# 0xPabloxx/3d-pointcloud-orientation-estimation

Measured on AMD Instinct MI355X. Metric: clouds/sec fwd+bwd, pointnet_pp_vonMises N=1024, higher is better.
Workload: dtype f32; 1 GPU; configs[1]: models/pointnet_pp_vonMises.py single-peak KL, N=1024, batch=32 per GPU, fwd+loss+bwd+allreduce+Adam, random-init weights (seed 42), device-side centre sampling; per_gpu_batch=32, global_batch=32, points=1024, parallelism=single, launch=hipGraph(fwd+loss+bwd) + eager all-reduce/Adam (the update clears the gradients)

## Files before the change

### 3d-pointcloud-orientation-estimation_amd/csrc/gemm_kernels.hip

```cpp
#include <stdlib.h>

#include "kernels.h"

namespace pnpp {

static bool mid_tiles_on() {
    static int cached = -1;
    if (cached < 0) {
        const char *v = getenv("PNPP_NO_MID");
        cached = (v && atoi(v) != 0) ? 0 : 1;
    }
    return cached != 0;
}

constexpr int KC = 32;
constexpr int APITCH = KC + 1;

struct RawA {
    float4 p, q;
    int4 ia;
};

template <int MODE>
__device__ __forceinline__ RawA fetch_a4(const AOperand &A, int row, int k, int M, int Kd) {
// ... 1052 lines not shown
                        }
                        if constexpr (DEFER) held = acc[i][j], held_m0 = m0;
                        if constexpr (EMODE == E_STORE_STATS) s1[j] += (double)t1, s2[j] += (double)t2;
                        if constexpr (EMODE == E_STORE_STATS) {
                            if (E.pool_ext) {
                                const float sg = pool_sg[j];
                                float mx = sg * acc[i][j][0];
#pragma unroll
                                for (int r = 1; r < 16; ++r) mx = fmaxf(mx, sg * acc[i][j][r]);
                                mx = fmaxf(mx, __shfl_xor(mx, 32, 64));
                                int a = 64;
#pragma unroll
                                for (int r = 15; r >= 0; --r) a = (sg * acc[i][j][r] == mx) ? (r & 3) + 8 * (r >> 2) + 4 * lh : a;
                                a = min(a, __shfl_xor(a, 32, 64));
                                if constexpr (DEFER) {
                                    held_ext = sg * mx, held_arg = a;
                                } else if (lh == 0) {
                                    const size_t gi = (size_t)((m0 + wm * TM + i * 32) >> 5) * E.ldc + (n0 + wn * TN + j * 32 + l31);
                                    E.pool_ext[gi] = sg * mx;
                                    E.pool_arg[gi] = a;
                                }
                            }
                        }
                    }
            }
        }
        if constexpr (EMODE == E_MASK_STATS && NT == 1) {
            if (m0 + BM <= M && n0 + BN <= Nout) {
                done = true;
#pragma unroll
                for (int i = 0; i < MT; ++i)
#pragma unroll
                    for (int j = 0; j < NT; ++j) {
                        const int col = n0 + wn * TN + j * 32 + l31;
                        const float sc = E.scale[col], sh = E.shift[col], mu = E.mu[col], is = E.istd[col];
                        float *tb = E.c + (size_t)(m0 + wm * TM + i * 32) * E.ldc + (n0 + wn * TN + j * 32);
                        const unsigned lo = (unsigned)(4 * lh) * (unsigned)E.ldc + (unsigned)l31;
                        float *apb = Ap + (wm * TM + i * 32 + 4 * lh) * BN + wn * TN + j * 32 + l31;
                        float t1 = 0.f, t2 = 0.f;
#pragma unroll
                        for (int r = 0; r < 16; ++r) {
                            const float z0 = zp[i][j][r];
                            const float a0 = fmaf(z0, sc, sh);
                            const float v = a0 > 0.f ? acc[i][j][r] : 0.f;
                            float *tr = tb + (size_t)((r & 3) + 8 * (r >> 2)) * E.ldc;
                            if (!PNPP_WS_EXP_NO_STORE) tr[lo] = v;
                            t1 += v;
                            t2 = fmaf(v, (z0 - mu) * is, t2);
                            if constexpr (FDW) apb[((r & 3) + 8 * (r >> 2)) * BN] = fmaxf(a0, 0.f);
                        }
                        s1[j] += (double)t1, s2[j] += (double)t2;
                    }
            }
        }
        if (!done)
#pragma unroll
        for (int i = 0; i < MT; ++i)
#pragma unroll
            for (int j = 0; j < NT; ++j) {
                const int col = n0 + wn * TN + j * 32 + l31;
                float sc = 0.f, sh = 0.f, mu = 0.f, is = 0.f;
                if constexpr (EMODE == E_MASK_STATS) {
                    const int cc = min(col, Nout - 1);
                    sc = E.scale[cc], sh = E.shift[cc], mu = E.mu[cc], is = E.istd[cc];
                }
                float t1 = 0.f, t2 = 0.f;
#pragma unroll
                for (int r = 0; r < 16; ++r) {
                    const int row = m0 + wm * TM + i * 32 + (r & 3) + 8 * (r >> 2) + 4 * lh;
                    const bool ok = row < M && col < Nout;
                    float v = ok ? acc[i][j][r] : 0.f;
                    if constexpr (EMODE == E_STORE_STATS) {
                        t1 += v;
                        t2 = fmaf(v, v, t2);
                    } else if constexpr (EMODE == E_MASK_STATS) {
                        const float z0 = zp[i][j][r];
                        v = (fmaf(z0, sc, sh) > 0.f) ? v : 0.f;
                        t1 += v;
                        t2 = fmaf(v, (z0 - mu) * is, t2);
                    }
                    if (ok) E.c[(size_t)row * E.ldc + col] = v;
                    if constexpr (FDW) {
                        const int rl = wm * TM + i * 32 + (r & 3) + 8 * (r >> 2) + 4 * lh;
                        Ap[rl * BN + wn * TN + j * 32 + l31] = fmaxf(fmaf(zp[i][j][r], sc, sh), 0.f);
                    }
                }
                if constexpr (EMODE != E_STORE) s1[j] += (double)t1, s2[j] += (double)t2;
            }
        PNPP_STAMP(5)
        if constexpr (FDW) {
            __syncthreads();
            PNPP_STAMP(6)
            static_assert(4 % (BN / 32) == 0, "a wave's dW tiles must share their activation columns");
            constexpr int MC = BM / 32;
            const int kt = wave % (BN / 32);
            int colx[DT];
#pragma unroll
            for (int t = 0; t < DT; ++t) colx[t] = (((wave + 4 * t) / (BN / 32)) * 32 + l31) ^ (lh << 2);
            const float *abase = As + lh * KP, *bbase = Ap + lh * BN + kt * 32 + l31;
            float da[2][MC][DT], db[2][MC];
            auto ld = [&](int buf, int t2) {
                const int F = (t2 & 7) << 3;
                const float *pb = bbase + 2 * t2 * BN;
#pragma unroll
                for (int c = 0; c < MC; ++c) db[buf][c] = pb[32 * c * BN];
#pragma unroll
                for (int t = 0; t < DT; ++t) {
                    const float *pa = abase + 2 * t2 * KP + (colx[t] ^ F);
#pragma unroll
                    for (int c = 0; c < MC; ++c) da[buf][c][t] = pa[32 * c * KP];
                }
            };
            auto mm = [&](int buf) {
#pragma unroll
                for (int c = 0; c < MC; ++c)
#pragma unroll
                    for (int t = 0; t < DT; ++t)
                        dwacc[t] = PNPP_WS_MFMA(da[buf][c][t], db[buf][c], dwacc[t]);
            };
            if constexpr (KD >= PNPP_WS_DWTABLE_MINK || TUNED_128) {
                const float *pre[DT][8];
#pragma unroll
                for (int t = 0; t < DT; ++t)
#pragma unroll
                    for (int f = 0; f < 8; ++f) pre[t][f] = abase + 2 * f * KP + (colx[t] ^ (f << 3));
                auto ldt = [&](int buf, int t2) {
                    const int f = t2 & 7, h = t2 >> 3;
                    const float *pb = bbase + 2 * t2 * BN;
#pragma unroll
                    for (int c = 0; c < MC; ++c) db[buf][c] = pb[32 * c * BN];
#pragma unroll
                    for (int t = 0; t < DT; ++t) {
                        const float *pa = pre[t][f] + 16 * h * KP;
#pragma unroll
                        for (int c = 0; c < MC; ++c) da[buf][c][t] = pa[32 * c * KP];
                    }
                };
                ldt(0, 0);
#pragma unroll
                for (int t2 = 0; t2 < 16; t2 += 2) {
                    ldt(1, t2 + 1);
                    mm(0);
                    if (t2 + 2 < 16) ldt(0, t2 + 2);
                    mm(1);
                }
            } else {
                ld(0, 0);
#pragma unroll 1
                for (int t2 = 0; t2 < 16; t2 += 2) {
                    ld(1, t2 + 1);
                    mm(0);
                    if (t2 + 2 < 16) ld(0, t2 + 2);
                    mm(1);
                }
            }
            PNPP_STAMP(7)
        }
    }

    flush_held();
    PNPP_STAMP(9)
    if constexpr (FDW) {
      if (n0 + BN <= Nout) {
        float *wb = E.dwslab + (size_t)worker * KD * E.dw_ld + n0;
        const unsigned lo = (unsigned)(4 * lh) * (unsigned)E.dw_ld + (unsigned)l31;
#pragma unroll
        for (int t = 0; t < DT; ++t) {
            const int tile_id = wave + 4 * t, ct = tile_id / (BN / 32), kt = tile_id % (BN / 32);
            float *tb = wb + (size_t)(ct * 32) * E.dw_ld + kt * 32;
#pragma unroll
            for (int r = 0; r < 16; ++r) tb[(size_t)((r & 3) + 8 * (r >> 2)) * E.dw_ld + lo] = dwacc[t][r];
        }
      } else
#pragma unroll
        for (int t = 0; t < DT; ++t) {
            const int tile_id = wave + 4 * t, ct = tile_id / (BN / 32), kt = tile_id % (BN / 32);
#pragma unroll
            for (int r = 0; r < 16; ++r) {
                const int c = ct * 32 + (r & 3) + 8 * (r >> 2) + 4 * lh, k = n0 + kt * 32 + l31;
                if (k < Nout) E.dwslab[((size_t)worker * KD + c) * E.dw_ld + k] = dwacc[t][r];
            }
        }
    }

    if constexpr (EMODE != E_STORE) {
        __syncthreads();
        double *red = reinterpret_cast<double *>(lds);
#pragma unroll
        for (int j = 0; j < NT; ++j) {
            double a = s1[j] + shfl_xor_f64(s1[j], 32);
            double b = s2[j] + shfl_xor_f64(s2[j], 32);
            if (lh == 0) {
                const int cl = wn * TN + j * 32 + l31;
                red[(wm * 2 + 0) * BN + cl] = a;
                red[(wm * 2 + 1) * BN + cl] = b;
            }
        }
        __syncthreads();
        for (int f = tid; f < 2 * BN; f += 256) {
            const int which = f / BN, cl = f % BN;
            double t = 0.0;
#pragma unroll
            for (int w = 0; w < WM; ++w) t += red[(w * 2 + which) * BN + cl];
            if (n0 + cl < Nout) E.slab[((size_t)worker * 2 + which) * Nout + n0 + cl] = t;
        }
    }
    PNPP_STAMP(10)
}

template <int KD, int BM, int BN, int WM, int WN, int AM, int EM, bool FDW>
static int launch_ws_one(const AOperand &A, const BOperand &B, int M, int Nout, const Epilogue &E, int *nslab, hipStream_t st,
                         int *dw_slabs) {
    const int tiles = cdiv(M, BM), ncol = cdiv(Nout, BN);
    size_t lds = ((size_t)KD * BN + (size_t)BM * (KD % 32 == 0 ? KD : KD + 1) + (FDW ? (size_t)BM * BN : 0)) * sizeof(float);
    const size_t red_bytes = (size_t)WM * 2 * BN * sizeof(double);
    if (lds < red_bytes) lds = red_bytes;
    int per_cu = (int)((160 * 1024) / lds);
    if (per_cu > 3) per_cu = 3;
    if (per_cu < 1) per_cu = 1;
    int workers = (256 * per_cu) / ncol;
    if (workers > tiles) workers = tiles;
    if (workers > kMaxStatBlocks) workers = kMaxStatBlocks;
    if (workers < 1) workers = 1;
    if (nslab) *nslab = workers;
    if (dw_slabs) *dw_slabs = FDW ? workers : 0;
    ProfScope ps(st, "gemm_ws_kernel<%d,%d,%d,A%d,E%d%s> M=%d N=%d K=%d grid=%dx1", KD, BM, BN, AM, EM, FDW ? ",dW" : "", M, Nout,
                 KD, workers * ncol);
    auto kfn = gemm_ws_kernel<KD, BM, BN, WM, WN, AM, EM, FDW>;
    static size_t lds_granted = 0;
    if (lds > 48 * 1024 && lds > lds_granted) {
        (void)hipFuncSetAttribute((const void *)kfn, hipFuncAttributeMaxDynamicSharedMemorySize, (int)lds);
        lds_granted = lds;
    }
    hipLaunchKernelGGL(kfn, dim3(workers * ncol), dim3(256), lds, st, A, B, M, Nout, ncol, E);
    PNPP_CHECK_LAUNCH("gemm_ws");
    return PNPP_OK;
}

template <int KD, int BM, int BN, int WM, int WN, int AM>
static int launch_ws_e(const AOperand &A, const BOperand &B, int M, int Nout, const Epilogue &E, int *nslab, hipStream_t st,
                       int *dw_slabs = nullptr) {
    if (dw_slabs) *dw_slabs = 0;
    switch (E.mode) {
        case E_STORE: return launch_ws_one<KD, BM, BN, WM, WN, AM, E_STORE, false>(A, B, M, Nout, E, nslab, st, nullptr);
        case E_STORE_STATS: return launch_ws_one<KD, BM, BN, WM, WN, AM, E_STORE_STATS, false>(A, B, M, Nout, E, nslab, st, nullptr);
        case E_MASK_STATS:
            if constexpr ((AM == A_DZ || AM == A_DZ_POOL) && KD % 32 == 0 && ((KD / 32) * (BN / 32)) % 4 == 0) {
                if (E.dwslab && dw_slabs)
                    return launch_ws_one<KD, BM, BN, WM, WN, AM, E_MASK_STATS, true>(A, B, M, Nout, E, nslab, st, dw_slabs);
            }
            return launch_ws_one<KD, BM, BN, WM, WN, AM, E_MASK_STATS, false>(A, B, M, Nout, E, nslab, st, nullptr);
    }
    set_error("gemm_ws: bad epilogue mode %d", E.mode);
    return PNPP_ERR_ARG;
}

template <int KD, int BM, int BN, int WM, int WN>
static int launch_ws_dense(const AOperand &A, const BOperand &B, int M, int Nout, const Epilogue &E, int *nslab, hipStream_t st,
                           int *dw_slabs) {
    switch (A.mode) {
        case A_PLAIN: return launch_ws_e<KD, BM, BN, WM, WN, A_PLAIN>(A, B, M, Nout, E, nslab, st);
        case A_BNRELU: return launch_ws_e<KD, BM, BN, WM, WN, A_BNRELU>(A, B, M, Nout, E, nslab, st);
        case A_DZ: return launch_ws_e<KD, BM, BN, WM, WN, A_DZ>(A, B, M, Nout, E, nslab, st, dw_slabs);
        case A_DZ_POOL: return launch_ws_e<KD, BM, BN, WM, WN, A_DZ_POOL>(A, B, M, Nout, E, nslab, st, dw_slabs);
    }
    set_error("gemm_ws: bad A mode %d", A.mode);
    return PNPP_ERR_ARG;
}

static bool try_launch_ws(const AOperand &A, const BOperand &B, int M, int Nout, int Kd, const Epilogue &E, int *nslab,
                          hipStream_t st, int *rc, int *dw_slabs) {
    if (M < 8192 || Nout % 64 != 0) return false;
    const bool grouped = A.mode == A_GATHER || A.mode == A_CONCAT;
    if (grouped) {
        if (Kd != A.D + 4) return false;
        if (A.mode != A_GATHER) return false;
        if (A.D == 0) {
            if (Nout % 128 == 0) *rc = launch_ws_e<4, 128, 128, 4, 1, A_GATHER>(A, B, M, Nout, E, nslab, st);
            else *rc = launch_ws_e<4, 128, 64, 4, 1, A_GATHER>(A, B, M, Nout, E, nslab, st);
            return true;
        }
        if (A.D == 128 && ((uintptr_t)A.a & 15) == 0) {
            *rc = launch_ws_e<132, 64, 64, 2, 2, A_GATHER>(A, B, M, Nout, E, nslab, st);
            return true;
        }
        return false;
    }
    if (A.lda % 4 != 0 || ((uintptr_t)A.a & 15) != 0) return false;
    if (Kd == 64) {
        *rc = launch_ws_dense<64, 64, 64, 2, 2>(A, B, M, Nout, E, nslab, st, dw_slabs);
        return true;
    }
    if (Kd == 128) {
        *rc = launch_ws_dense<128, 64, 64, 2, 2>(A, B, M, Nout, E, nslab, st, dw_slabs);
        return true;
    }
    if (Kd == 256) {
        *rc = launch_ws_dense<256, 64, 64, 2, 2>(A, B, M, Nout, E, nslab, st, dw_slabs);
        return true;
    }
    return false;
}

template <int AMODE, int EMODE, bool BT, int NW>
__device__ __forceinline__ void gemm_smallm_body(const AOperand &A, const BOperand &B, int M, int Nout, int Kd, const Epilogue &E,
                                                 int bx, int by, int nblocks) {
    constexpr int NTHR = NW * 64, NJ = 1024 / NTHR;
    __shared__ __attribute__((aligned(16))) float lds[2 * NW * 32 * APITCH];
    const int tid = threadIdx.x, lane = tid & 63, wave = tid >> 6, l31 = lane & 31, lh = lane >> 5;
    float *As = lds + wave * 32 * APITCH;
    float *Ws = lds + (NW + wave) * 32 * APITCH;
    float *part = lds;
    const float *__restrict__ Bm = B.b;
    const int ldb = B.ldb;
    const int n0 = bx * 32, m0 = by * 32;
    const int nchunks = (Kd + KC - 1) / KC;
    const bool bvec = (ldb & 3) == 0 && ((uintptr_t)Bm & 15) == 0 && B.perm_D < 0 && B.rows >= 4 && (B.rows & 3) == 0;

    f32x16 acc;
#pragma unroll
    for (int r = 0; r < 16; ++r) acc[r] = 0.f;

    float p_g = 1.f, p_b = 0.f, p_bias = 0.f, p_rm = 0.f, p_rv = 0.f;
    unsigned long long p_sid = 0ull;
    if constexpr (EMODE == E_BN_APPLY) {
        const BnTail &T = E.bn;
        if (tid < 32 && n0 + tid < Nout) {
            const int c = n0 + tid;
            if (T.gamma) p_g = T.gamma[c];
            if (T.beta) p_b = T.beta[c];
            if (T.bias) p_bias = T.bias[c];
            if (T.rm) p_rm = T.rm[c], p_rv = T.rv[c];
        }
        if (T.mask_out) p_sid = T.rng_counter[0];
    }

    RawA na[4];
    float4 nw[4];
    float nb[KC / 2];
    auto fetch = [&](int c) {
        const int k0 = c * KC;
#pragma unroll
        for (int i = 0; i < 4; ++i) {
            const int r = (lane >> 3) + 8 * i, k = k0 + 4 * (lane & 7);
            na[i] = fetch_a4<AMODE>(A, m0 + r, k, M, Kd);
            if constexpr (BT) {
                const float *wrow = Bm + (size_t)min(n0 + r, Nout - 1) * ldb;
                if (bvec) {
                    nw[i] = *reinterpret_cast<const float4 *>(wrow + min(k, B.rows - 4));
                } else {
                    float t[4];
#pragma unroll
                    for (int e = 0; e < 4; ++e) {
                        const int kp = min(k + e, B.rows - 1);
                        t[e] = wrow[B.perm_D >= 0 ? (kp < B.perm_D ? kp + 3 : kp - B.perm_D) : kp];
                    }
                    nw[i] = make_float4(t[0], t[1], t[2], t[3]);
                }
            }
        }
        if constexpr (!BT) {
#pragma unroll
            for (int s2 = 0; s2 < KC / 2; ++s2) {
                const int k = k0 + 2 * s2 + lh;
                const float v = Bm[(size_t)min(k, B.rows - 1) * ldb + min(n0 + l31, Nout - 1)];
                nb[s2] = v * ((k < B.rows && n0 + l31 < Nout) ? 1.f : 0.f);
            }
        }
    };
    if (wave < nchunks) fetch(wave);
    for (int c = wave; c < nchunks; c += NW) {
        float cb[KC / 2];
        const int k0 = c * KC;
#pragma unroll
        for (int i = 0; i < 4; ++i) {
            const int r = (lane >> 3) + 8 * i, k = k0 + 4 * (lane & 7);
            const int o = r * APITCH + 4 * (lane & 7);
            float v[4];
            xform_a4<AMODE>(A, na[i], m0 + r, k, M, Kd, v);
            As[o] = v[0], As[o + 1] = v[1], As[o + 2] = v[2], As[o + 3] = v[3];
            if constexpr (BT) {
                const bool okw = n0 + r < Nout;
                Ws[o] = (okw && k < B.rows) ? nw[i].x : 0.f;
                Ws[o + 1] = (okw && k + 1 < B.rows) ? nw[i].y : 0.f;
                Ws[o + 2] = (okw && k + 2 < B.rows) ? nw[i].z : 0.f;
                Ws[o + 3] = (okw && k + 3 < B.rows) ? nw[i].w : 0.f;
            }
        }
        if constexpr (!BT) {
#pragma unroll
            for (int s2 = 0; s2 < KC / 2; ++s2) cb[s2] = nb[s2];
        }
        if (c + NW < nchunks) fetch(c + NW);
#pragma unroll
        for (int s2 = 0; s2 < KC / 2; ++s2) {
            const float bv = BT ? Ws[l31 * APITCH + 2 * s2 + lh] : cb[s2];
            acc = __builtin_amdgcn_mfma_f32_32x32x2f32(As[l31 * APITCH + 2 * s2 + lh], bv, acc, 0, 0, 0);
        }
    }
#pragma unroll
    for (int r = 0; r < 16; ++r) part[wave * 32 * APITCH + ((r & 3) + 8 * (r >> 2) + 4 * lh) * 32 + l31] = acc[r];
    __syncthreads();
    float v[NJ], w2[NJ];
#pragma unroll
    for (int j = 0; j < NJ; ++j) {
        const int e = tid + NTHR * j;
        v[j] = 0.f;
#pragma unroll
        for (int w = 0; w < NW; w += 4)
            v[j] += (part[w * 32 * APITCH + e] + part[(w + 1) * 32 * APITCH + e]) +
                    (part[(w + 2) * 32 * APITCH + e] + part[(w + 3) * 32 * APITCH + e]);
        w2[j] = 0.f;
    }
    __syncthreads();
#pragma unroll
    for (int j = 0; j < NJ; ++j) {
        const int e = tid + NTHR * j, row = m0 + e / 32, col = n0 + e % 32;
        const bool ok = row < M && col < Nout;
        float x = ok ? v[j] : 0.f;
        if constexpr (EMODE == E_MASK_STATS) {
            const int cc = min(col, Nout - 1);
            const float zp = E.zp[(size_t)min(row, M - 1) * E.ldc + cc];
            x = (fmaf(zp, E.scale[cc], E.shift[cc]) > 0.f) ? x : 0.f;
            w2[j] = x * ((zp - E.mu[cc]) * E.istd[cc]);
            part[1024 + e] = w2[j];
        }
        part[e] = x;
        if (ok) E.c[(size_t)row * E.ldc + col] = x;
    }
    if constexpr (EMODE == E_BN_APPLY) {
        const BnTail &T = E.bn;
        float *cs = part + 2048;
        __syncthreads();
        if (tid < 32 && n0 + tid < Nout) {
            const int c = n0 + tid;
            double s1 = 0.0, s2 = 0.0;
            for (int r = 0; r < 32; ++r) {
                const double x = (double)part[r * 32 + tid];
                s1 += x;
                s2 += x * x;
            }
            const double count = (double)M;
            const double mu = s1 / count;
            double var = s2 / count - mu * mu;
            if (var < 0.0) var = 0.0;
            const double is = 1.0 / sqrt(var + (double)T.eps);
            const double g = (double)p_g, bt = (double)p_b;
            const float sc = (float)(g * is), sh = (float)(bt - mu * g * is);
            T.mean[c] = (float)mu;
            T.istd[c] = (float)is;
            T.scale[c] = sc;
            T.shift[c] = sh;
            cs[tid] = sc;
            cs[32 + tid] = sh;
            if (T.rm) {
                const double bmean = mu + (double)p_bias;
                const double unbiased = count > 1.0 ? var * count / (count - 1.0) : var;
                T.rm[c] = (float)((1.0 - (double)T.momentum) * (double)p_rm + (double)T.momentum * bmean);
                T.rv[c] = (float)((1.0 - (double)T.momentum) * (double)p_rv + (double)T.momentum * unbiased);
            }
        }
        if (T.nbt && bx == 0 && tid == 0) *T.nbt += 1;
        __syncthreads();
#pragma unroll
        for (int j = 0; j < NJ; ++j) {
            const int e = tid + NTHR * j, row = m0 + e / 32, col = n0 + e % 32;
            if (row < M && col < Nout) {
                float y = fmaf(part[e], cs[e % 32], cs[32 + e % 32]);
                if (T.relu) y = fmaxf(y, 0.f);
                if (T.mask) y = T.mask[(size_t)row * E.ldc + col] ? y * T.drop_scale : 0.f;
                if (T.mask_out) {
                    const unsigned long long sid = p_sid;
                    const unsigned idx = (unsigned)(row * E.ldc + col);
                    unsigned c0 = idx, c1 = 0x44524f50u , c2 = (unsigned)sid, c3 = (unsigned)(sid >> 32);
                    unsigned k0 = (unsigned)T.rng_seed, k1 = (unsigned)(T.rng_seed >> 32);
#pragma unroll
                    for (int rd = 0; rd < 10; ++rd) {
                        const unsigned long long p0 = (unsigned long long)0xD2511F53u * c0, p1 = (unsigned long long)0xCD9E8D57u * c2;
                        const unsigned n0 = (unsigned)(p1 >> 32) ^ c1 ^ k0, n1 = (unsigned)p1, n2 = (unsigned)(p0 >> 32) ^ c3 ^ k1, n3 = (unsigned)p0;
                        c0 = n0, c1 = n1, c2 = n2, c3 = n3;
                        k0 += 0x9E3779B9u, k1 += 0xBB67AE85u;
                    }
                    const bool keep = (double)c0 >= (double)T.drop_p * 4294967296.0;
                    T.mask_out[(size_t)row * E.ldc + col] = keep ? 1 : 0;
                    y = keep ? y * T.drop_scale : 0.f;
                }
                T.y[(size_t)row * E.ldc + col] = y;
            }
        }
        if (T.mask_out) {
            __syncthreads();
            if (tid == 0) {
                const unsigned long long t = atomicAdd(&T.rng_counter[1], 1ull);
                if (t == (unsigned long long)nblocks - 1) {
                    T.rng_counter[1] = 0ull;
                    T.rng_counter[0] += 1ull;
                }
            }
        }
    } else if constexpr (EMODE != E_STORE) {
        __syncthreads();
        if (tid < 32 && n0 + tid < Nout) {
            double s1 = 0.0, s2 = 0.0;
            for (int r = 0; r < 32; ++r) {
                const double x = (double)part[r * 32 + tid];
                s1 += x;
                if constexpr (EMODE == E_STORE_STATS) s2 += x * x;
                else s2 += (double)part[1024 + r * 32 + tid];
            }
            E.slab[((size_t)by * 2 + 0) * Nout + n0 + tid] = s1;
            E.slab[((size_t)by * 2 + 1) * Nout + n0 + tid] = s2;
        }
    }
}

template <int AMODE, int EMODE, bool BT, int NW>
__global__ void __launch_bounds__(NW * 64)
gemm_smallm_kernel(const AOperand A, const BOperand B, int M, int Nout, int Kd, const Epilogue E) {
    gemm_smallm_body<AMODE, EMODE, BT, NW>(A, B, M, Nout, Kd, E, blockIdx.x, blockIdx.y, gridDim.x * gridDim.y);
}

template <int AM, int EM>
static void launch_smallm_t(const AOperand &A, const BOperand &B, int M, int Nout, int Kd, const Epilogue &E, dim3 grid,
                            hipStream_t st) {
    if constexpr (AM == A_PLAIN) {
        if (grid.y == 1 && Kd >= 256) {
            if (B.trans) hipLaunchKernelGGL((gemm_smallm_kernel<AM, EM, true, 16>), grid, dim3(1024), 0, st, A, B, M, Nout, Kd, E);
            else hipLaunchKernelGGL((gemm_smallm_kernel<AM, EM, false, 16>), grid, dim3(1024), 0, st, A, B, M, Nout, Kd, E);
            return;
        }
    }
    if (B.trans) hipLaunchKernelGGL((gemm_smallm_kernel<AM, EM, true, 4>), grid, dim3(256), 0, st, A, B, M, Nout, Kd, E);
    else hipLaunchKernelGGL((gemm_smallm_kernel<AM, EM, false, 4>), grid, dim3(256), 0, st, A, B, M, Nout, Kd, E);
}
template <int AM>
static int launch_smallm_e(const AOperand &A, const BOperand &B, int M, int Nout, int Kd, const Epilogue &E, dim3 grid,
                           hipStream_t st) {
    switch (E.mode) {
        case E_STORE: launch_smallm_t<AM, E_STORE>(A, B, M, Nout, Kd, E, grid, st); return PNPP_OK;
        case E_STORE_STATS: launch_smallm_t<AM, E_STORE_STATS>(A, B, M, Nout, Kd, E, grid, st); return PNPP_OK;
        case E_MASK_STATS: launch_smallm_t<AM, E_MASK_STATS>(A, B, M, Nout, Kd, E, grid, st); return PNPP_OK;
        case E_BN_APPLY:
            if constexpr (AM == A_PLAIN) {
                PNPP_REQUIRE(grid.y == 1 && E.bn.mean && E.bn.istd && E.bn.scale && E.bn.shift && E.bn.y, PNPP_ERR_ARG,
                             "gemm(small M): the BatchNorm epilogue needs all rows in one tile (M <= 32) and its outputs");
                launch_smallm_t<AM, E_BN_APPLY>(A, B, M, Nout, Kd, E, grid, st);
                return PNPP_OK;
            }
            break;
    }
    set_error("gemm(small M): bad epilogue mode %d", E.mode);
    return PNPP_ERR_ARG;
}

template <int BM, int BN, int WM, int WN>
static int launch_gemm_cfg(const AOperand &A, const BOperand &B, int M, int Nout, int Kd, const Epilogue &E, int *nslab,
                           hipStream_t st) {
    const int tiles = cdiv(M, BM);
    const int gx = tiles < kMaxStatBlocks ? tiles : kMaxStatBlocks;
    const dim3 grid(gx, cdiv(Nout, BN)), block(WM * WN * 64);
    if (nslab) *nslab = gx;
    ProfScope ps(st, "gemm_kernel<%d,%d,%d,%d,A%d,E%d> M=%d N=%d K=%d grid=%dx%d", BM, BN, WM, WN, A.mode, E.mode, M, Nout, Kd,
                 grid.x, grid.y);
#define PNPP_LAUNCH(AM, EM)                                                                                   \
    hipLaunchKernelGGL((gemm_kernel<BM, BN, WM, WN, AM, EM>), grid, block, 0, st, A, B, M, Nout, Kd, E); \
    break;
#define PNPP_BY_E(AM)                                                          \
    switch (E.mode) {                                                          \
        case E_STORE: PNPP_LAUNCH(AM, E_STORE)                                 \
        case E_STORE_STATS: PNPP_LAUNCH(AM, E_STORE_STATS)                     \
        case E_MASK_STATS: PNPP_LAUNCH(AM, E_MASK_STATS)                       \
        default: set_error("gemm: bad epilogue mode %d", E.mode); return PNPP_ERR_ARG; \
    }                                                                          \
    break;
    switch (A.mode) {
        case A_PLAIN: PNPP_BY_E(A_PLAIN)
        case A_BNRELU: PNPP_BY_E(A_BNRELU)
        case A_GATHER: PNPP_BY_E(A_GATHER)
        case A_CONCAT: PNPP_BY_E(A_CONCAT)
        case A_DZ: PNPP_BY_E(A_DZ)
        case A_DZ_POOL: PNPP_BY_E(A_DZ_POOL)
        default: set_error("gemm: bad A mode %d", A.mode); return PNPP_ERR_ARG;
    }
#undef PNPP_BY_E
#undef PNPP_LAUNCH
    PNPP_CHECK_LAUNCH("gemm");
    return PNPP_OK;
}

bool gemm_pools_in_epilogue(const AOperand &A, int M, int Nout, int Kd, int nsample) {
    if (nsample != 32) return false;
    if (M < 8192) return mid_tiles_on() && mid_gemm_pools(A, M, Nout, Kd);
    if (matmul_precision() != 0) return false;
    if (M % 64 != 0 || Nout % 64 != 0) return false;
    if (!(A.mode == A_PLAIN || A.mode == A_BNRELU)) return false;
    if (A.lda % 4 != 0 || ((uintptr_t)A.a & 15) != 0) return false;
    return Kd == 64 || Kd == 128 || Kd == 256;
}

int launch_gemm(const AOperand &A, const BOperand &Bin, int M, int Nout, int Kd, const Epilogue &E, int *nslab,
                hipStream_t st, int *dw_slabs) {
    if (dw_slabs) *dw_slabs = 0;
    PNPP_REQUIRE(M > 0 && Nout > 0 && Kd > 0, PNPP_ERR_ARG, "gemm: non-positive size M=%d N=%d K=%d", M, Nout, Kd);
    PNPP_REQUIRE(Bin.b && Bin.ldb > 0, PNPP_ERR_ARG, "gemm: null B operand");
    PNPP_REQUIRE(Kd % 4 == 0, PNPP_ERR_ARG, "gemm: K=%d must be a multiple of 4", Kd);
    BOperand B = Bin;
    if (B.rows <= 0 || B.rows > Kd) B.rows = Kd;
    {
        int rc = PNPP_OK;
        if (try_launch_ws_bf16(A, B, M, Nout, Kd, E, nslab, st, &rc, dw_slabs)) return rc;
        if (try_launch_wsf3(A, B, M, Nout, Kd, E, nslab, st, &rc)) return rc;
        if (try_launch_wsf(A, B, M, Nout, Kd, E, nslab, st, &rc)) return rc;
        if (try_launch_wsd3(A, B, M, Nout, Kd, E, nslab, st, &rc, dw_slabs)) return rc;
        if (try_launch_wsp(A, B, M, Nout, Kd, E, nslab, st, &rc, dw_slabs)) return rc;
        if (try_launch_wsq(A, B, M, Nout, Kd, E, nslab, st, &rc, dw_slabs)) return rc;
        if (try_launch_ws(A, B, M, Nout, Kd, E, nslab, st, &rc, dw_slabs)) return rc;
        if (mid_tiles_on() && try_launch_mid_gemm(A, B, M, Nout, Kd, E, nslab, st, &rc)) return rc;
    }
    const bool a_aligned = (A.mode == A_CONCAT || A.mode == A_GATHER) || (A.lda % 4 == 0 && ((uintptr_t)A.a & 15) == 0);
    if (M <= 4096 && cdiv(M, 32) <= kMaxStatBlocks && a_aligned && A.mode != A_GATHER) {
        const dim3 grid(cdiv(Nout, 32), cdiv(M, 32));
        if (nslab) *nslab = grid.y;
        ProfScope ps(st, "gemm_smallm_kernel<A%d,E%d,T%d> M=%d N=%d K=%d grid=%dx%d", A.mode, E.mode, B.trans, M, Nout, Kd, grid.x,
                     grid.y);
        int rc = PNPP_OK;
        switch (A.mode) {
            case A_PLAIN: rc = launch_smallm_e<A_PLAIN>(A, B, M, Nout, Kd, E, grid, st); break;
            case A_BNRELU: rc = launch_smallm_e<A_BNRELU>(A, B, M, Nout, Kd, E, grid, st); break;
            case A_CONCAT: rc = launch_smallm_e<A_CONCAT>(A, B, M, Nout, Kd, E, grid, st); break;
            case A_DZ: rc = launch_smallm_e<A_DZ>(A, B, M, Nout, Kd, E, grid, st); break;
            case A_DZ_POOL: rc = launch_smallm_e<A_DZ_POOL>(A, B, M, Nout, Kd, E, grid, st); break;
            default: set_error("gemm(small M): bad A mode %d", A.mode); return PNPP_ERR_ARG;
        }
        if (rc != PNPP_OK) return rc;
        PNPP_CHECK_LAUNCH("gemm(small M)");
        return PNPP_OK;
    }
    if (A.mode == A_PLAIN || A.mode == A_BNRELU || A.mode == A_DZ || A.mode == A_DZ_POOL)
        PNPP_REQUIRE(A.lda % 4 == 0 && ((uintptr_t)A.a & 15) == 0, PNPP_ERR_ARG, "gemm: A operand pitch/alignment");
    if (M >= 128 * 128) {
        if (Nout % 128 == 0) return launch_gemm_cfg<128, 128, 4, 2>(A, B, M, Nout, Kd, E, nslab, st);
        if (Nout % 64 == 0) return launch_gemm_cfg<128, 64, 4, 2>(A, B, M, Nout, Kd, E, nslab, st);
        return launch_gemm_cfg<128, 32, 4, 1>(A, B, M, Nout, Kd, E, nslab, st);
    }
    if (M > 32) {
        if (Nout % 64 == 0) return launch_gemm_cfg<64, 64, 2, 2>(A, B, M, Nout, Kd, E, nslab, st);
        return launch_gemm_cfg<128, 32, 4, 1>(A, B, M, Nout, Kd, E, nslab, st);
    }
    if (Nout % 128 == 0) return launch_gemm_cfg<32, 128, 1, 4>(A, B, M, Nout, Kd, E, nslab, st);
    return launch_gemm_cfg<128, 32, 4, 1>(A, B, M, Nout, Kd, E, nslab, st);
}

template <int MODE>
__global__ void __launch_bounds__(256) dz_materialize_kernel(const AOperand A, int M, int C, float *__restrict__ out) {
    const size_t total = (size_t)M * (C / 4);
    for (size_t i = (size_t)blockIdx.x * 256 + threadIdx.x; i < total; i += (size_t)gridDim.x * 256) {
        const int row = (int)(i / (C / 4)), k = 4 * (int)(i % (C / 4));
        const RawA r = fetch_a4<MODE>(A, row, k, M, C);
        float v[4];
        xform_a4<MODE>(A, r, row, k, M, C, v);
        *reinterpret_cast<float4 *>(out + (size_t)row * C + k) = make_float4(v[0], v[1], v[2], v[3]);
    }
}

int launch_dz_materialize(const AOperand &dz, int M, int C, float *out, hipStream_t st) {
    PNPP_REQUIRE(C % 4 == 0 && (dz.mode == A_DZ || dz.mode == A_DZ_POOL), PNPP_ERR_ARG, "dz_materialize: bad operand");
    const size_t total = (size_t)M * (C / 4);
    const int grid = (int)((total + 255) / 256 < 2048 ? (total + 255) / 256 : 2048);
    ProfScope ps(st, "dz_materialize_kernel M=%d C=%d", M, C);
    if (dz.mode == A_DZ) hipLaunchKernelGGL(dz_materialize_kernel<A_DZ>, dim3(grid), dim3(256), 0, st, dz, M, C, out);
    else hipLaunchKernelGGL(dz_materialize_kernel<A_DZ_POOL>, dim3(grid), dim3(256), 0, st, dz, M, C, out);
    PNPP_CHECK_LAUNCH("dz_materialize");
    return PNPP_OK;
}

template <int DZMODE, int A2MODE, int CT, int KT>
__global__ void __launch_bounds__(256)
dw_kernel(const AOperand dz, const AOperand a2, int M, int Nc, int Kp, int tilesC, int tilesK, int rows_per_split,
          int kp_pad, float *__restrict__ slab) {
    constexpr int U = 4;
    const int lane = threadIdx.x & 63, l31 = lane & 31, lh = lane >> 5;
    const int gw = blockIdx.x * 4 + (threadIdx.x >> 6);
    const int tiles = tilesC * tilesK;
    const int tile = gw % tiles, split = gw / tiles;
    const int r0 = min(M, split * rows_per_split);
    const int r1 = min(M, r0 + rows_per_split);
    const int c0 = (tile % tilesC) * 32 * CT, k0 = (tile / tilesC) * 32 * KT;

    ChanConst cc[CT], ck[KT];
#pragma unroll
    for (int i = 0; i < CT; ++i) cc[i] = load_chan_const<DZMODE>(dz, c0 + i * 32 + l31, Nc);
#pragma unroll
    for (int j = 0; j < KT; ++j) ck[j] = load_chan_const<A2MODE>(a2, k0 + j * 32 + l31, Kp);

    f32x16 acc[CT][KT];
#pragma unroll
    for (int i = 0; i < CT; ++i)
#pragma unroll
        for (int j = 0; j < KT; ++j)
#pragma unroll
            for (int r = 0; r < 16; ++r) acc[i][j][r] = 0.f;

    const bool grp_batch = (DZMODE == A_DZ_POOL) && (dz.K % (2 * U) == 0) && (r0 % (2 * U) == 0);
    for (int row = r0; row < r1; row += 2 * U) {
        float2 fa[U][CT], fb[U][KT];
        float gdm[CT];
        int garg[CT], gk0 = 0;
        if (DZMODE == A_DZ_POOL && grp_batch) {
            const int g = row / dz.K;
            gk0 = row - g * dz.K;
#pragma unroll
            for (int i = 0; i < CT; ++i) {
                const int c = min(c0 + i * 32 + l31, Nc - 1);
                gdm[i] = dz.a[(size_t)g * dz.lda + c];
                garg[i] = dz.arg[(size_t)g * dz.lda + c];
            }
        }
#pragma unroll
        for (int u = 0; u < U; ++u) {
            const int m = row + 2 * u + lh;
#pragma unroll
            for (int i = 0; i < CT; ++i) {
                if (DZMODE == A_DZ_POOL && grp_batch) {
                    const int c = min(c0 + i * 32 + l31, Nc - 1);
                    fa[u][i].x = (gk0 + 2 * u + lh == garg[i]) ? gdm[i] : 0.f;
                    fa[u][i].y = dz.z[(size_t)min(m, M - 1) * dz.lda + c];
                } else {
                    fa[u][i] = fetch_a1<DZMODE>(dz, m, c0 + i * 32 + l31, Nc, M);
                }
            }
#pragma unroll
            for (int j = 0; j < KT; ++j) fb[u][j] = fetch_a1<A2MODE>(a2, m, k0 + j * 32 + l31, Kp, M);
        }
#pragma unroll
        for (int u = 0; u < U; ++u) {
            const bool ok = row + 2 * u + lh < r1;
            float a[CT], b[KT];
#pragma unroll
            for (int i = 0; i < CT; ++i) a[i] = xform_a1<DZMODE>(fa[u][i], cc[i], c0 + i * 32 + l31, Nc, ok);
#pragma unroll
            for (int j = 0; j < KT; ++j) b[j] = xform_a1<A2MODE>(fb[u][j], ck[j], k0 + j * 32 + l31, Kp, ok);
#pragma unroll
            for (int i = 0; i < CT; ++i)
#pragma unroll
                for (int j = 0; j < KT; ++j)
                    acc[i][j] = __builtin_amdgcn_mfma_f32_32x32x2f32(a[i], b[j], acc[i][j], 0, 0, 0);
        }
    }
    float *o = slab + (size_t)split * Nc * kp_pad;
#pragma unroll
    for (int i = 0; i < CT; ++i)
#pragma unroll
        for (int j = 0; j < KT; ++j)
#pragma unroll
            for (int r = 0; r < 16; ++r) {
                const int c = c0 + i * 32 + (r & 3) + 8 * (r >> 2) + 4 * lh;
                const int k = k0 + j * 32 + l31;
                if (c < Nc && k < kp_pad) o[(size_t)c * kp_pad + k] = acc[i][j][r];
            }
}

template <int DZMODE, int A2MODE>
__global__ void __launch_bounds__(256)
dw_xyz_kernel(const AOperand dz, const AOperand a2, int M, int C, float *__restrict__ slab) {
    __shared__ float rel[256][4];
    __shared__ float red[4][64][3];
    const int tid = threadIdx.x, cl = tid & 63, rl = tid >> 6;
    const int m0 = blockIdx.x * 256;
    {
        const float2 x = fetch_a1<A2MODE>(a2, m0 + tid, 0, 3, M);
        const float2 y = fetch_a1<A2MODE>(a2, m0 + tid, 1, 3, M);
        const float2 z = fetch_a1<A2MODE>(a2, m0 + tid, 2, 3, M);
        const float okf = (m0 + tid < M) ? 1.f : 0.f;
        rel[tid][0] = __fsub_rn(x.x, x.y) * okf;
        rel[tid][1] = __fsub_rn(y.x, y.y) * okf;
        rel[tid][2] = __fsub_rn(z.x, z.y) * okf;
        rel[tid][3] = 0.f;
    }
    __syncthreads();
    for (int c0 = blockIdx.y * 64; c0 < C; c0 += gridDim.y * 64) {
        const int c = c0 + cl;
        const ChanConst cc = load_chan_const<DZMODE>(dz, min(c, C - 1), C);
        float a0 = 0.f, a1 = 0.f, a2s = 0.f;
#pragma unroll 8
        for (int r = rl; r < 256; r += 4) {
            const float2 f = fetch_a1<DZMODE>(dz, m0 + r, c, C, M);
            const float g = xform_a1<DZMODE>(f, cc, c, C, true);
            const float4 q = *reinterpret_cast<const float4 *>(rel[r]);
            a0 = fmaf(g, q.x, a0), a1 = fmaf(g, q.y, a1), a2s = fmaf(g, q.z, a2s);
        }
        red[rl][cl][0] = a0, red[rl][cl][1] = a1, red[rl][cl][2] = a2s;
        __syncthreads();
        if (tid < 192) {
            const int ch = tid / 3, k = tid - 3 * ch;
            if (c0 + ch < C)
                slab[((size_t)blockIdx.x * C + c0 + ch) * 4 + k] = (red[0][ch][k] + red[1][ch][k]) + (red[2][ch][k] + red[3][ch][k]);
        }
        __syncthreads();
    }
}

int dw_xyz_splits(int M) { return cdiv(M, 256); }

template <int A2MODE>
static int launch_dw_xyz_a2(const AOperand &dz, int C, const AOperand &a2, int M, float *slab, dim3 grid, hipStream_t st) {
    switch (dz.mode) {
        case A_PLAIN: hipLaunchKernelGGL((dw_xyz_kernel<A_PLAIN, A2MODE>), grid, dim3(256), 0, st, dz, a2, M, C, slab); break;
        case A_DZ: hipLaunchKernelGGL((dw_xyz_kernel<A_DZ, A2MODE>), grid, dim3(256), 0, st, dz, a2, M, C, slab); break;
        case A_DZ_POOL: hipLaunchKernelGGL((dw_xyz_kernel<A_DZ_POOL, A2MODE>), grid, dim3(256), 0, st, dz, a2, M, C, slab); break;
        default: set_error("dw_xyz: bad dZ mode %d", dz.mode); return PNPP_ERR_ARG;
    }
    return PNPP_OK;
}

int launch_dw_xyz(const AOperand &dz, int C, const AOperand &a2, int M, float *slab, hipStream_t st) {
    PNPP_REQUIRE((a2.mode == A_GATHER || a2.mode == A_CONCAT) && a2.D == 0, PNPP_ERR_ARG,
                 "dw_xyz: the second operand must be xyz-only (gathered or whole-cloud)");
    PNPP_REQUIRE(M > 0 && C > 0, PNPP_ERR_ARG, "dw_xyz: non-positive size");
    const dim3 grid(dw_xyz_splits(M), 1);
    ProfScope ps(st, "dw_xyz_kernel<A%d,A%d> M=%d N=%d K=3 grid=%dx1", dz.mode, a2.mode, M, C, grid.x);
    const int rc = a2.mode == A_GATHER ? launch_dw_xyz_a2<A_GATHER>(dz, C, a2, M, slab, grid, st)
                                       : launch_dw_xyz_a2<A_CONCAT>(dz, C, a2, M, slab, grid, st);
    if (rc != PNPP_OK) return rc;
    PNPP_CHECK_LAUNCH("dw_xyz");
    return PNPP_OK;
}

__global__ void __launch_bounds__(256)
gather_rel_stats_kernel(const float *__restrict__ P, const float *__restrict__ xyz, const float *__restrict__ new_xyz,
                        const int32_t *__restrict__ idx, const float *__restrict__ W0, int ldw, int N, int S, int K, int M,
                        int C, int rpb, float *__restrict__ z, double *__restrict__ slab) {
    extern __shared__ __attribute__((aligned(16))) double gred[];
    const int LPR = C >> 2, RPP = 256 / LPR;
    const int cl = threadIdx.x % LPR, rl = threadIdx.x / LPR, c4 = cl * 4;
    float wx[4], wy[4], wz[4];
#pragma unroll
    for (int e = 0; e < 4; ++e) {
        const float *w = W0 + (size_t)(c4 + e) * ldw;
        wx[e] = w[0], wy[e] = w[1], wz[e] = w[2];
    }
    const int r0 = blockIdx.x * rpb, r1 = min(M, r0 + rpb);
    double d1[4] = {0.0, 0.0, 0.0, 0.0}, d2[4] = {0.0, 0.0, 0.0, 0.0};
    for (int rb = r0 + rl; rb < r1; rb += 4 * RPP) {
        float4 p[4];
        float rx[4], ry[4], rz[4], ok[4];
#pragma unroll
        for (int u = 0; u < 4; ++u) {
            const int r = rb + u * RPP;
            const int rc = min(r, r1 - 1);
            ok[u] = r < r1 ? 1.f : 0.f;
            const int grp = rc / K;
            const size_t src = (size_t)(grp / S) * N + idx[rc];
            p[u] = *reinterpret_cast<const float4 *>(P + src * C + c4);
            const float *x = xyz + src * 3, *c = new_xyz + (size_t)grp * 3;
            rx[u] = __fsub_rn(x[0], c[0]), ry[u] = __fsub_rn(x[1], c[1]), rz[u] = __fsub_rn(x[2], c[2]);
        }
        float s1[4] = {0.f, 0.f, 0.f, 0.f}, s2[4] = {0.f, 0.f, 0.f, 0.f};
#pragma unroll
        for (int u = 0; u < 4; ++u) {
            float v[4] = {p[u].x, p[u].y, p[u].z, p[u].w};
#pragma unroll
            for (int e = 0; e < 4; ++e) {
                v[e] = fmaf(rz[u], wz[e], fmaf(ry[u], wy[e], fmaf(rx[u], wx[e], v[e])));
                const float m = v[e] * ok[u];
                s1[e] += m, s2[e] = fmaf(m, m, s2[e]);
            }
            const int r = rb + u * RPP;
            if (r < r1) *reinterpret_cast<float4 *>(z + (size_t)r * C + c4) = make_float4(v[0], v[1], v[2], v[3]);
        }
#pragma unroll
        for (int e = 0; e < 4; ++e) d1[e] += (double)s1[e], d2[e] += (double)s2[e];
    }
    if (slab == nullptr) return;
#pragma unroll
    for (int e = 0; e < 4; ++e) {
        gred[(rl * 2 + 0) * C + c4 + e] = d1[e];
        gred[(rl * 2 + 1) * C + c4 + e] = d2[e];
    }
    __syncthreads();
    for (int f = threadIdx.x; f < 2 * C; f += 256) {
        const int which = f / C, c = f - which * C;
        double t = 0.0;
        for (int w = 0; w < RPP; ++w) t += gred[(w * 2 + which) * C + c];
        slab[((size_t)blockIdx.x * 2 + which) * C + c] = t;
    }
}

bool delayed_layer0_ok(int C) {
    return C >= 32 && C <= 512 && (C & (C - 1)) == 0;
}

int launch_gather_rel_stats(const float *P, const AOperand &geo, const float *W0, int ldw, int M, int C, float *z,
                            double *slab, int *nslab, hipStream_t st) {
    PNPP_REQUIRE(delayed_layer0_ok(C) && geo.mode == A_GATHER, PNPP_ERR_ARG, "gather_rel_stats: unsupported width %d", C);
    const int rpp = 256 / (C / 4);
    int rpb = 64;
    while (rpb < 4 * rpp || cdiv(M, rpb) > kMaxStatBlocks) rpb *= 2;
    const int grid = cdiv(M, rpb);
    if (nslab) *nslab = grid;
    ProfScope ps(st, "gather_rel_stats_kernel M=%d C=%d grid=%d", M, C, grid);
    hipLaunchKernelGGL(gather_rel_stats_kernel, dim3(grid), dim3(256), (size_t)rpp * 2 * C * sizeof(double), st, P, geo.xyz,
                       geo.new_xyz, geo.idx, W0, ldw, geo.N, geo.S, geo.K, M, C, rpb, z, slab);
    PNPP_CHECK_LAUNCH("gather_rel_stats");
    return PNPP_OK;
}

constexpr int SCW = 8;
constexpr int SCWIN = 1024;
template <int NCH>
__global__ void __launch_bounds__(SCW * 64)
scatter_dz_kernel(const AOperand dz, const AOperand geo, int Mc, int C, int total, float *__restrict__ G,
                  float *__restrict__ wslab) {
    constexpr int UB = NCH == 1 ? 8 : 4;
    __shared__ int hl[SCW][SCWIN];
    __shared__ float wred[SCW][NCH * 128][3];
    const int lane = threadIdx.x & 63, wv = threadIdx.x >> 6;
    const int N = geo.N;
    const int dst = min(blockIdx.x * SCW + wv, total - 1);
    const bool live = blockIdx.x * SCW + wv < total;
    const int b = dst / N, n = dst - b * N;
    const int32_t *ib = geo.idx + (size_t)b * Mc;
    const size_t row0 = (size_t)b * Mc;
    const float px = geo.xyz[(size_t)dst * 3], py = geo.xyz[(size_t)dst * 3 + 1], pz = geo.xyz[(size_t)dst * 3 + 2];
    const float *cb = geo.new_xyz + (size_t)b * geo.S * 3;
    float2 cg[NCH], cmu[NCH], cis[NCH], c1[NCH], c2[NCH], acc[NCH], ax[NCH], ay[NCH], az[NCH];
    int cc[NCH];
#pragma unroll
    for (int j = 0; j < NCH; ++j) {
        cc[j] = min(j * 128 + 2 * lane, C - 2);
        cg[j] = make_float2(1.f, 1.f);
// ... 1062 lines not shown
```

Before: 60290 clouds/s.

## Add narrow-column small-M GEMM kernel for head layers with split-K MFMA

Adds a specialised kernel for the classifier-head GEMMs (M<=32, K>=256, transposed B) that gives each block only 8 output columns. Inside the block, 16 waves split K and each runs 16x16x4 f32 MFMAs, then the partial tiles are reduced through LDS. The aim is to spread these skinny head GEMMs over more workgroups so the GPU is better occupied. The BatchNorm tail is factored into shared helpers so the new kernel reuses it. The trade-off is extra LDS reduction work and a larger grid.

```diff
diff --git a/3d-pointcloud-orientation-estimation_amd/csrc/gemm_kernels.hip b/3d-pointcloud-orientation-estimation_amd/csrc/gemm_kernels.hip
--- a/3d-pointcloud-orientation-estimation_amd/csrc/gemm_kernels.hip
+++ b/3d-pointcloud-orientation-estimation_amd/csrc/gemm_kernels.hip
@@ -1378,6 +1378,66 @@
     return false;
 }
 
+__device__ __forceinline__ void bn_tail_column(const BnTail &T, const float *colp, int pitch, int M, int c, float p_g, float p_b,
+                                               float p_bias, float p_rm, float p_rv, float &sc_out, float &sh_out) {
+    double s1 = 0.0, s2 = 0.0;
+    for (int r = 0; r < 32; ++r) {
+        const double x = (double)colp[r * pitch];
+        s1 += x;
+        s2 += x * x;
+    }
+    const double count = (double)M;
+    const double mu = s1 / count;
+    double var = s2 / count - mu * mu;
+    if (var < 0.0) var = 0.0;
+    const double is = 1.0 / sqrt(var + (double)T.eps);
+    const double g = (double)p_g, bt = (double)p_b;
+    const float sc = (float)(g * is), sh = (float)(bt - mu * g * is);
+    T.mean[c] = (float)mu;
+    T.istd[c] = (float)is;
+    T.scale[c] = sc;
+    T.shift[c] = sh;
+    sc_out = sc;
+    sh_out = sh;
+    if (T.rm) {
+        const double bmean = mu + (double)p_bias;
+        const double unbiased = count > 1.0 ? var * count / (count - 1.0) : var;
+        T.rm[c] = (float)((1.0 - (double)T.momentum) * (double)p_rm + (double)T.momentum * bmean);
+        T.rv[c] = (float)((1.0 - (double)T.momentum) * (double)p_rv + (double)T.momentum * unbiased);
+    }
+}
+
+__device__ __forceinline__ void bn_tail_apply(const BnTail &T, float z, float sc, float sh, int row, int col, int ldc,
+                                              unsigned long long sid) {
+    float y = fmaf(z, sc, sh);
+    if (T.relu) y = fmaxf(y, 0.f);
+    if (T.mask) y = T.mask[(size_t)row * ldc + col] ? y * T.drop_scale : 0.f;
+    if (T.mask_out) {
+        const unsigned idx = (unsigned)(row * ldc + col);
+        unsigned c0 = idx, c1 = 0x44524f50u , c2 = (unsigned)sid, c3 = (unsigned)(sid >> 32);
+        unsigned k0 = (unsigned)T.rng_seed, k1 = (unsigned)(T.rng_seed >> 32);
+#pragma unroll
+        for (int rd = 0; rd < 10; ++rd) {
+            const unsigned long long p0 = (unsigned long long)0xD2511F53u * c0, p1 = (unsigned long long)0xCD9E8D57u * c2;
+            const unsigned n0 = (unsigned)(p1 >> 32) ^ c1 ^ k0, n1 = (unsigned)p1, n2 = (unsigned)(p0 >> 32) ^ c3 ^ k1, n3 = (unsigned)p0;
+            c0 = n0, c1 = n1, c2 = n2, c3 = n3;
+            k0 += 0x9E3779B9u, k1 += 0xBB67AE85u;
+        }
+        const bool keep = (double)c0 >= (double)T.drop_p * 4294967296.0;
+        T.mask_out[(size_t)row * ldc + col] = keep ? 1 : 0;
+        y = keep ? y * T.drop_scale : 0.f;
+    }
+    T.y[(size_t)row * ldc + col] = y;
+}
+
+__device__ __forceinline__ void bn_tail_ticket(const BnTail &T, int nblocks) {
+    const unsigned long long t = atomicAdd(&T.rng_counter[1], 1ull);
+    if (t == (unsigned long long)nblocks - 1) {
+        T.rng_counter[1] = 0ull;
+        T.rng_counter[0] += 1ull;
+    }
+}
+
 template <int AMODE, int EMODE, bool BT, int NW>
 __device__ __forceinline__ void gemm_smallm_body(const AOperand &A, const BOperand &B, int M, int Nout, int Kd, const Epilogue &E,
                                                  int bx, int by, int nblocks) {
@@ -1509,32 +1569,7 @@
         float *cs = part + 2048;
         __syncthreads();
         if (tid < 32 && n0 + tid < Nout) {
-            const int c = n0 + tid;
-            double s1 = 0.0, s2 = 0.0;
-            for (int r = 0; r < 32; ++r) {
-                const double x = (double)part[r * 32 + tid];
-                s1 += x;
-                s2 += x * x;
-            }
-            const double count = (double)M;
-            const double mu = s1 / count;
-            double var = s2 / count - mu * mu;
-            if (var < 0.0) var = 0.0;
-            const double is = 1.0 / sqrt(var + (double)T.eps);
-            const double g = (double)p_g, bt = (double)p_b;
-            const float sc = (float)(g * is), sh = (float)(bt - mu * g * is);
-            T.mean[c] = (float)mu;
-            T.istd[c] = (float)is;
-            T.scale[c] = sc;
-            T.shift[c] = sh;
-            cs[tid] = sc;
-            cs[32 + tid] = sh;
-            if (T.rm) {
-                const double bmean = mu + (double)p_bias;
-                const double unbiased = count > 1.0 ? var * count / (count - 1.0) : var;
-                T.rm[c] = (float)((1.0 - (double)T.momentum) * (double)p_rm + (double)T.momentum * bmean);
-                T.rv[c] = (float)((1.0 - (double)T.momentum) * (double)p_rv + (double)T.momentum * unbiased);
-            }
+            bn_tail_column(T, part + tid, 32, M, n0 + tid, p_g, p_b, p_bias, p_rm, p_rv, cs[tid], cs[32 + tid]);
         }
         if (T.nbt && bx == 0 && tid == 0) *T.nbt += 1;
         __syncthreads();
@@ -1542,37 +1577,12 @@
         for (int j = 0; j < NJ; ++j) {
             const int e = tid + NTHR * j, row = m0 + e / 32, col = n0 + e % 32;
             if (row < M && col < Nout) {
-                float y = fmaf(part[e], cs[e % 32], cs[32 + e % 32]);
-                if (T.relu) y = fmaxf(y, 0.f);
-                if (T.mask) y = T.mask[(size_t)row * E.ldc + col] ? y * T.drop_scale : 0.f;
-                if (T.mask_out) {
-                    const unsigned long long sid = p_sid;
-                    const unsigned idx = (unsigned)(row * E.ldc + col);
-                    unsigned c0 = idx, c1 = 0x44524f50u , c2 = (unsigned)sid, c3 = (unsigned)(sid >> 32);
-                    unsigned k0 = (unsigned)T.rng_seed, k1 = (unsigned)(T.rng_seed >> 32);
-#pragma unroll
-                    for (int rd = 0; rd < 10; ++rd) {
-                        const unsigned long long p0 = (unsigned long long)0xD2511F53u * c0, p1 = (unsigned long long)0xCD9E8D57u * c2;
-                        const unsigned n0 = (unsigned)(p1 >> 32) ^ c1 ^ k0, n1 = (unsigned)p1, n2 = (unsigned)(p0 >> 32) ^ c3 ^ k1, n3 = (unsigned)p0;
-                        c0 = n0, c1 = n1, c2 = n2, c3 = n3;
-                        k0 += 0x9E3779B9u, k1 += 0xBB67AE85u;
-                    }
-                    const bool keep = (double)c0 >= (double)T.drop_p * 4294967296.0;
-                    T.mask_out[(size_t)row * E.ldc + col] = keep ? 1 : 0;
-                    y = keep ? y * T.drop_scale : 0.f;
-                }
-                T.y[(size_t)row * E.ldc + col] = y;
+                bn_tail_apply(T, part[e], cs[e % 32], cs[32 + e % 32], row, col, E.ldc, p_sid);
             }
         }
         if (T.mask_out) {
             __syncthreads();
-            if (tid == 0) {
-                const unsigned long long t = atomicAdd(&T.rng_counter[1], 1ull);
-                if (t == (unsigned long long)nblocks - 1) {
-                    T.rng_counter[1] = 0ull;
-                    T.rng_counter[0] += 1ull;
-                }
-            }
+            if (tid == 0) bn_tail_ticket(T, nblocks);
         }
     } else if constexpr (EMODE != E_STORE) {
         __syncthreads();
@@ -1596,6 +1606,128 @@
     gemm_smallm_body<AMODE, EMODE, BT, NW>(A, B, M, Nout, Kd, E, blockIdx.x, blockIdx.y, gridDim.x * gridDim.y);
 }
 
+template <int EMODE, int NC, int NW>
+__global__ void __launch_bounds__(NW * 64)
+gemm_smallm_narrow_kernel(const AOperand A, const BOperand B, int M, int Nout, int Kd, const Epilogue E) {
+    static_assert((NC == 8 || NC == 16) && NW % 4 == 0 && 32 * NC <= NW * 64 && (EMODE == E_STORE || EMODE == E_BN_APPLY), "narrow head form");
+    constexpr int TILE = 32 * NC, UB = 2;
+    __shared__ __attribute__((aligned(16))) float part[NW * TILE];
+    __shared__ float tile[TILE];
+    __shared__ float cs[2 * NC];
+    const int tid = threadIdx.x, lane = tid & 63, wave = __builtin_amdgcn_readfirstlane(tid >> 6), l15 = lane & 15, q = lane >> 4;
+    const int n0 = blockIdx.x * NC;
+    const int nunits = (Kd + 15) / 16;
+    const float *__restrict__ a0 = A.a + (size_t)min(l15, M - 1) * A.lda;
+    const float *__restrict__ a1 = A.a + (size_t)min(16 + l15, M - 1) * A.lda;
+    const float *__restrict__ wp = B.b + (size_t)min(n0 + (l15 & (NC - 1)), Nout - 1) * B.ldb;
+
+    float p_g = 1.f, p_b = 0.f, p_bias = 0.f, p_rm = 0.f, p_rv = 0.f;
+    unsigned long long p_sid = 0ull;
+    if constexpr (EMODE == E_BN_APPLY) {
+        const BnTail &T = E.bn;
+        if (tid < NC && n0 + tid < Nout) {
+            const int c = n0 + tid;
+            if (T.gamma) p_g = T.gamma[c];
+            if (T.beta) p_b = T.beta[c];
+            if (T.bias) p_bias = T.bias[c];
+            if (T.rm) p_rm = T.rm[c], p_rv = T.rv[c];
+        }
+        if (T.mask_out) p_sid = T.rng_counter[0];
+    }
+
+    f32x4 acc0 = {0.f, 0.f, 0.f, 0.f}, acc1 = {0.f, 0.f, 0.f, 0.f};
+    struct Batch { float4 x0[UB], x1[UB], w[UB]; } s0, s1;
+    auto fetch = [&](int b, Batch &s) {
+#pragma unroll
+        for (int i = 0; i < UB; ++i) {
+            const int k = 16 * (wave + NW * (b * UB + i)) + 4 * q;
+            const int ka = min(k, Kd - 4);
+            s.x0[i] = *reinterpret_cast<const float4 *>(a0 + ka);
+            s.x1[i] = *reinterpret_cast<const float4 *>(a1 + ka);
+            s.w[i] = *reinterpret_cast<const float4 *>(wp + min(k, B.rows - 4));
+        }
+    };
+    auto mac = [&](int b, const Batch &s) {
+#pragma unroll
+        for (int i = 0; i < UB; ++i) {
+            if (wave + NW * (b * UB + i) < nunits) {
+                const int k = 16 * (wave + NW * (b * UB + i)) + 4 * q;
+                const float m = (k < Kd && k < B.rows) ? 1.f : 0.f;
+                const float xa[4] = {s.x0[i].x, s.x0[i].y, s.x0[i].z, s.x0[i].w}, xb[4] = {s.x1[i].x, s.x1[i].y, s.x1[i].z, s.x1[i].w};
+                const float wv[4] = {s.w[i].x * m, s.w[i].y * m, s.w[i].z * m, s.w[i].w * m};
+#pragma unroll
+                for (int e = 0; e < 4; ++e) {
+                    acc0 = __builtin_amdgcn_mfma_f32_16x16x4f32(xa[e], wv[e], acc0, 0, 0, 0);
+                    acc1 = __builtin_amdgcn_mfma_f32_16x16x4f32(xb[e], wv[e], acc1, 0, 0, 0);
+                }
+            }
+        }
+    };
+    const int nbatch = (nunits - wave + NW * UB - 1) / (NW * UB);
+    auto pass = [&](int b) {
+        const bool two = b + 1 < nbatch;
+        fetch(b, s0);
+        if (two) fetch(b + 1, s1);
+        mac(b, s0);
+        if (two) mac(b + 1, s1);
+    };
+    pass(0);
+    for (int b = 2; b < nbatch; b += 2) pass(b);
+    if (l15 < NC) {
+#pragma unroll
+        for (int r = 0; r < 4; ++r) {
+            part[wave * TILE + (4 * q + r) * NC + l15] = acc0[r];
+            part[wave * TILE + (16 + 4 * q + r) * NC + l15] = acc1[r];
+        }
+    }
+    __syncthreads();
+    const int row = tid / NC, col = n0 + tid % NC;
+    const bool mine = tid < TILE, ok = mine && row < M && col < Nout;
+    if (mine) {
+        float v = 0.f;
+#pragma unroll
+        for (int w = 0; w < NW; w += 4)
+            v += (part[w * TILE + tid] + part[(w + 1) * TILE + tid]) + (part[(w + 2) * TILE + tid] + part[(w + 3) * TILE + tid]);
+        const float x = ok ? v : 0.f;
+        tile[tid] = x;
+        if (ok) E.c[(size_t)row * E.ldc + col] = x;
+    }
+    if constexpr (EMODE == E_BN_APPLY) {
+        const BnTail &T = E.bn;
+        __syncthreads();
+        if (tid < NC && n0 + tid < Nout) {
+            asm volatile("" : "+v"(p_rm), "+v"(p_rv));
+            bn_tail_column(T, tile + tid, NC, M, n0 + tid, p_g, p_b, p_bias, p_rm, p_rv, cs[tid], cs[NC + tid]);
+        }
+        if (T.nbt && blockIdx.x == 0 && tid == 0) *T.nbt += 1;
+        __syncthreads();
+        if (ok) bn_tail_apply(T, tile[tid], cs[tid % NC], cs[NC + tid % NC], row, col, E.ldc, p_sid);
+        if (T.mask_out) {
+            __syncthreads();
+            if (tid == 0) bn_tail_ticket(T, (int)gridDim.x);
+        }
+    }
+}
+
+#ifndef PNPP_HEAD_NARROW_COLS
+#define PNPP_HEAD_NARROW_COLS 8
+#endif
+static_assert(PNPP_HEAD_NARROW_COLS == 0 || PNPP_HEAD_NARROW_COLS == 8 || PNPP_HEAD_NARROW_COLS == 16, "PNPP_HEAD_NARROW_COLS");
+
+static int head_narrow_cols(const AOperand &A, const BOperand &B, int M, int Kd, const Epilogue &E) {
+    if (A.mode != A_PLAIN || M > 32 || Kd < 256 || !B.trans || B.perm_D >= 0) return 0;
+    if (E.mode != E_STORE && E.mode != E_BN_APPLY) return 0;
+    if ((B.ldb & 3) != 0 || ((uintptr_t)B.b & 15) != 0 || B.rows < 4 || (B.rows & 3) != 0) return 0;
+    return PNPP_HEAD_NARROW_COLS;
+}
+
+template <int EM>
+static void launch_smallm_narrow(const AOperand &A, const BOperand &B, int M, int Nout, int Kd, const Epilogue &E, int nc, hipStream_t st) {
+    const dim3 grid(cdiv(Nout, nc));
+    if (nc == 16) hipLaunchKernelGGL((gemm_smallm_narrow_kernel<EM, 16, 16>), grid, dim3(1024), 0, st, A, B, M, Nout, Kd, E);
+    else hipLaunchKernelGGL((gemm_smallm_narrow_kernel<EM, 8, 16>), grid, dim3(1024), 0, st, A, B, M, Nout, Kd, E);
+}
+
 template <int AM, int EM>
 static void launch_smallm_t(const AOperand &A, const BOperand &B, int M, int Nout, int Kd, const Epilogue &E, dim3 grid,
                             hipStream_t st) {
@@ -1611,16 +1743,20 @@
 }
 template <int AM>
 static int launch_smallm_e(const AOperand &A, const BOperand &B, int M, int Nout, int Kd, const Epilogue &E, dim3 grid,
-                           hipStream_t st) {
+                           hipStream_t st, int narrow = 0) {
     switch (E.mode) {
-        case E_STORE: launch_smallm_t<AM, E_STORE>(A, B, M, Nout, Kd, E, grid, st); return PNPP_OK;
+        case E_STORE:
+            if (narrow) launch_smallm_narrow<E_STORE>(A, B, M, Nout, Kd, E, narrow, st);
+            else launch_smallm_t<AM, E_STORE>(A, B, M, Nout, Kd, E, grid, st);
+            return PNPP_OK;
         case E_STORE_STATS: launch_smallm_t<AM, E_STORE_STATS>(A, B, M, Nout, Kd, E, grid, st); return PNPP_OK;
         case E_MASK_STATS: launch_smallm_t<AM, E_MASK_STATS>(A, B, M, Nout, Kd, E, grid, st); return PNPP_OK;
         case E_BN_APPLY:
             if constexpr (AM == A_PLAIN) {
                 PNPP_REQUIRE(grid.y == 1 && E.bn.mean && E.bn.istd && E.bn.scale && E.bn.shift && E.bn.y, PNPP_ERR_ARG,
                              "gemm(small M): the BatchNorm epilogue needs all rows in one tile (M <= 32) and its outputs");
-                launch_smallm_t<AM, E_BN_APPLY>(A, B, M, Nout, Kd, E, grid, st);
+                if (narrow) launch_smallm_narrow<E_BN_APPLY>(A, B, M, Nout, Kd, E, narrow, st);
+                else launch_smallm_t<AM, E_BN_APPLY>(A, B, M, Nout, Kd, E, grid, st);
                 return PNPP_OK;
             }
             break;
@@ -1695,13 +1831,14 @@
     }
     const bool a_aligned = (A.mode == A_CONCAT || A.mode == A_GATHER) || (A.lda % 4 == 0 && ((uintptr_t)A.a & 15) == 0);
     if (M <= 4096 && cdiv(M, 32) <= kMaxStatBlocks && a_aligned && A.mode != A_GATHER) {
-        const dim3 grid(cdiv(Nout, 32), cdiv(M, 32));
+        const int narrow = head_narrow_cols(A, B, M, Kd, E);
+        const dim3 grid(cdiv(Nout, narrow ? narrow : 32), cdiv(M, 32));
         if (nslab) *nslab = grid.y;
         ProfScope ps(st, "gemm_smallm_kernel<A%d,E%d,T%d> M=%d N=%d K=%d grid=%dx%d", A.mode, E.mode, B.trans, M, Nout, Kd, grid.x,
                      grid.y);
         int rc = PNPP_OK;
         switch (A.mode) {
-            case A_PLAIN: rc = launch_smallm_e<A_PLAIN>(A, B, M, Nout, Kd, E, grid, st); break;
+            case A_PLAIN: rc = launch_smallm_e<A_PLAIN>(A, B, M, Nout, Kd, E, grid, st, narrow); break;
             case A_BNRELU: rc = launch_smallm_e<A_BNRELU>(A, B, M, Nout, Kd, E, grid, st); break;
             case A_CONCAT: rc = launch_smallm_e<A_CONCAT>(A, B, M, Nout, Kd, E, grid, st); break;
             case A_DZ: rc = launch_smallm_e<A_DZ>(A, B, M, Nout, Kd, E, grid, st); break;
```

New measurement: 60790 clouds/s, median of 6. No clear change (+0.8%).
